# phylo42/IPK

Hardware: AMD Instinct MI355X
Metric: scored phylo-k-mers/sec (higher is better)
Workload: dtype f32

## Files before the change

ipk_amd/csrc/ipkgpu.hip:

```cpp
#include <cstring>
#include <hip/hip_runtime.h>
#include <rocprim/rocprim.hpp>

#include <algorithm>
#include <cmath>
#include <cstdarg>
#include <cstdio>
#include <cstring>
#include <new>
#include <string>
#include <type_traits>
#include <unordered_map>
#include <memory>
#include <vector>

#include "../../include/ipkgpu.h"
#include "dcla_device.hpp"
#include "kernels_score.hpp"
#include "kernels_quad.hpp"
#include "kernels_compact.hpp"
#include "kernels_keymajor.hpp"
#include "kernels_reduce_pipe.hpp"
#include "kernels_filter.hpp"
#include "kernels_dbfile.hpp"
#include <chrono>

using namespace ipkgpu;


namespace {

struct DevBuf {
    void* p = nullptr;
    size_t cap = 0;
    template <class T> T* as() const { return reinterpret_cast<T*>(p); }
};

struct EventPool {
    std::vector<hipEvent_t> free_ev;
    hipEvent_t get()
    {
        if (!free_ev.empty()) { hipEvent_t e = free_ev.back(); free_ev.pop_back(); return e; }
        hipEvent_t e = nullptr;
        return hipEventCreate(&e) == hipSuccess ? e : nullptr;
    }
    void put(hipEvent_t e) { if (free_ev.size() < 64) free_ev.push_back(e); else (void)hipEventDestroy(e); }
};
struct Stopwatch {
    hipStream_t stream;
    EventPool* pool;
    std::vector<hipEvent_t> ev;
    Stopwatch(hipStream_t s, EventPool* p) : stream(s), pool(p) {}
    ~Stopwatch() { for (hipEvent_t e : ev) pool->put(e); }
    int mark()
    {
        hipEvent_t e = pool->get();
        if (!e) return -1;
        (void)hipEventRecord(e, stream);
        ev.push_back(e);
        return (int)ev.size() - 1;
    }
    double ms(int a, int b) const
    {
        float t = 0;
        if (a < 0 || b < 0 || hipEventElapsedTime(&t, ev[a], ev[b]) != hipSuccess) return 0;
        return t;
    }
};

}

struct ipkgpu_comm;
struct ipkgpu_ctx;
static void ipkgpu_comm_release(ipkgpu_ctx* ctx);
struct ipkgpu_ctx {
    int device = 0;
    ipkgpu_comm* comm = nullptr;
    hipStream_t stream = nullptr;
    std::string err;
    int64_t workspace_bytes = 0;
    int64_t opt_variant = 0;
    int64_t opt_flags = 0;
    int64_t opt_kmc_pass = 0;
    int64_t opt_prefix_mats = 0;
    int64_t opt_wg_chunks2 = 0;
    int64_t opt_rounds = 0;
    int64_t opt_pool_limit = 0;
    int64_t opt_pool_chunks = 0;
    DevBuf table, best, ovfq, counts, offsets, goff, idx, branch, scan_sums, scan_boff, tmp_a, tmp_b, tmp_c;
    DevBuf pool, desc, gbcnt, gboff, gbcur, clist, gm, tile_next;
    DevBuf ptrs;
    DevBuf mask;
    bool mask_valid = false;
    uint64_t mask_words = 0;
    bool table_compressed = false;
    DevBuf rank, vaddr, ucnt, qpack, xstart, pcounts;
    DevBuf cvals, coff, croom;
    bool comp_own_vals = false;
    std::vector<uint32_t> h_branch;
    uint32_t comp_nb = 0, comp_stride = 0, comp_tbl = 0;
    double pairs_per_window = 0;
    double acc_main_ms = 0, acc_reduce_ms = 0;
    double acc_count_ms = 0, acc_write_ms = 0, acc_km_ms = 0;
    const char* main_kernel = "";
    std::vector<std::pair<void*, size_t>> free_blocks;
    std::unordered_map<void*, size_t> live_blocks;
    size_t cached_bytes = 0, cache_limit = 0;
    void* small = nullptr;
    void* h_up = nullptr; size_t h_up_cap = 0; hipEvent_t up_done = nullptr; bool up_pending = false;
    unsigned long long emitted_host = 0; bool emitted_fetched = false;
    uint32_t* h_rb = nullptr;
    EventPool events;
    bool spec_skip_wait = false;
    uint64_t pool_want_min = 0;
    struct Pending {
        bool active = false;
        std::unique_ptr<Stopwatch> sw; int ev_a = -1, ev_b = -1, ev_c = -1, ev_d = -1;
        uint64_t cap = 0, max_chunks = 0, windows = 0; uint32_t gb = 0; bool pool_ovf_ok = false, use_quad = false;
    } pend;
    uint64_t last_entries = 0; uint32_t last_gb = 0;
    double t_write_total = 0, t_write_device = 0, t_write_file = 0;
    int num_cu = 256;
};

struct ipkgpu_result {
    ipkgpu_ctx* ctx = nullptr;
    std::vector<uint32_t> group_ids;
    std::vector<uint64_t> offsets;
    uint64_t emitted = 0;
    uint32_t* d_keys = nullptr;
    float* d_scores = nullptr;
    uint32_t* d_positions = nullptr;
    size_t cap = 0;
    std::vector<uint32_t> h_keys;
    std::vector<float> h_scores;
    std::vector<uint32_t> h_positions;
    bool h_keys_ok = false, h_scores_ok = false, h_positions_ok = false;
    double t_total = 0, t_prefix = 0, t_score = 0, t_compact = 0, t_main = 0, t_reduce = 0;
    int score_launches = 0;
};

struct ipkgpu_parts {
    ipkgpu_ctx* ctx = nullptr;
    uint32_t n_owners = 1;
    uint64_t slots = 0;
    uint32_t* d_counts = nullptr;
    uint2* d_entries = nullptr;
    std::vector<uint64_t> owner_off;
    uint64_t emitted = 0;
    uint32_t* pre_keys = nullptr; uint64_t* pre_key_off = nullptr; uint64_t pre_n_keys = 0; double t_keys = 0;
    uint32_t lead = 0;
    uint64_t key_base = 0;
    double t_total = 0, t_prefix = 0, t_score = 0, t_compact = 0, t_main = 0, t_reduce = 0, t_count = 0, t_write = 0, t_km = 0;
    int score_launches = 0;
};

struct ipkgpu_db {
    ipkgpu_ctx* ctx = nullptr;
    uint64_t n_keys = 0, n_entries = 0;
    uint32_t* d_keys = nullptr;
    uint64_t* d_key_off = nullptr;
    uint2* d_entries = nullptr;
    std::vector<uint32_t> h_keys;
    std::vector<uint64_t> h_key_off;
    std::vector<uint32_t> h_entries;
    bool h_ok = false;
    double t_merge = 0;
    double* d_fv64 = nullptr;
    float* d_fv32 = nullptr;
    uint32_t* d_order = nullptr;
    std::vector<double> h_fv64;
    std::vector<float> h_fv32;
    std::vector<uint32_t> h_order;
    bool h_filter_ok = false;
    double t_filter = 0;
};

static std::string g_create_err;
constexpr size_t RB_BYTES = 4096, RB_OWNER_OFF = 8 , RB_OWNERS_MAX = 500;

template <class T = uint32_t> static T* small_at(const ipkgpu_ctx* ctx, uint32_t off) { return reinterpret_cast<T*>(static_cast<char*>(ctx->small) + off); }

static int fail(ipkgpu_ctx* ctx, int code, const char* fmt, ...)
{
    char buf[512];
    va_list ap;
    va_start(ap, fmt);
    vsnprintf(buf, sizeof buf, fmt, ap);
    va_end(ap);
    if (ctx) ctx->err = buf; else g_create_err = buf;
    return code;
}

#define HIP_TRY(ctx, expr)                                                                      \
    do {                                                                                        \
        hipError_t e_ = (expr);                                                                 \
        if (e_ != hipSuccess)                                                                   \
            return fail(ctx, e_ == hipErrorOutOfMemory ? IPKGPU_ERR_NOMEM : IPKGPU_ERR_HIP,     \
                        "%s failed: %s (%s:%d)", #expr, hipGetErrorString(e_), __FILE__, __LINE__); \
    } while (0)
#define RC_TRY(expr) do { int rc_ = (expr); if (rc_) return rc_; } while (0)

static int ensure(ipkgpu_ctx* ctx, DevBuf& b, size_t need)
{
    if (b.cap >= need && b.p) return IPKGPU_OK;
    const bool regrow = b.p != nullptr;
    if (b.p) { HIP_TRY(ctx, hipFree(b.p)); b.p = nullptr; b.cap = 0; }
    need = std::max<size_t>(need, 16);
    size_t want = regrow ? need + need / 16 : need;
    hipError_t e = hipMalloc(&b.p, want);
    if (e != hipSuccess && want > need) { (void)hipGetLastError(); want = need; e = hipMalloc(&b.p, want); }
    HIP_TRY(ctx, e);
    b.cap = want;
    return IPKGPU_OK;
}


static int upload_stage(ipkgpu_ctx* ctx, size_t bytes, void** out)
{
    if (ctx->up_pending) { HIP_TRY(ctx, hipEventSynchronize(ctx->up_done)); ctx->up_pending = false; }
    if (!ctx->up_done) HIP_TRY(ctx, hipEventCreateWithFlags(&ctx->up_done, hipEventDisableTiming));
    if (bytes > ctx->h_up_cap) {
        if (ctx->h_up) { (void)hipHostFree(ctx->h_up); ctx->h_up = nullptr; ctx->h_up_cap = 0; }
        const size_t cap = std::max<size_t>(bytes + bytes / 2, 1 << 16);
        HIP_TRY(ctx, hipHostMalloc(&ctx->h_up, cap, hipHostMallocDefault));
        ctx->h_up_cap = cap;
    }
    *out = ctx->h_up;
    return IPKGPU_OK;
}
static int upload_staged(ipkgpu_ctx* ctx)
{
    HIP_TRY(ctx, hipEventRecord(ctx->up_done, ctx->stream));
    ctx->up_pending = true;
    return IPKGPU_OK;
}

static hipError_t ctx_alloc(ipkgpu_ctx* ctx, void** out, size_t bytes)
{
    bytes = std::max<size_t>((bytes + 255) & ~(size_t)255, 256);
    size_t best = (size_t)-1;
    for (size_t i = 0; i < ctx->free_blocks.size(); ++i) {
        const size_t cap = ctx->free_blocks[i].second;
        if (cap >= bytes && cap <= bytes + bytes / 2 + (1 << 20) && (best == (size_t)-1 || cap < ctx->free_blocks[best].second)) best = i;
    }
    if (best != (size_t)-1) {
        *out = ctx->free_blocks[best].first;
        ctx->live_blocks[*out] = ctx->free_blocks[best].second;
        ctx->cached_bytes -= ctx->free_blocks[best].second;
        ctx->free_blocks.erase(ctx->free_blocks.begin() + best);
        return hipSuccess;
    }
    hipError_t e = hipMalloc(out, bytes);
    if (e != hipSuccess && !ctx->free_blocks.empty()) {
        for (auto& b : ctx->free_blocks) (void)hipFree(b.first);
        ctx->free_blocks.clear(); ctx->cached_bytes = 0;
        (void)hipGetLastError();
        e = hipMalloc(out, bytes);
    }
    if (e == hipSuccess) ctx->live_blocks[*out] = bytes;
    return e;
}
static void ctx_release(ipkgpu_ctx* ctx, void* p)
{
    if (!p) return;
    auto it = ctx->live_blocks.find(p);
    if (it == ctx->live_blocks.end()) { (void)hipFree(p); return; }
    const size_t cap = it->second;
    ctx->live_blocks.erase(it);
    if (ctx->cached_bytes + cap <= ctx->cache_limit) { ctx->free_blocks.push_back({p, cap}); ctx->cached_bytes += cap; }
    else (void)hipFree(p);
}

static constexpr uint64_t WAVE_PER_ITEM_SPAN = 1ull << 24;

static hipError_t ctx_alloc_atleast(ipkgpu_ctx* ctx, void** out, size_t min_bytes, size_t want_bytes, size_t* got)
{
    min_bytes = std::max<size_t>((min_bytes + 255) & ~(size_t)255, 256);
    want_bytes = std::max(want_bytes, min_bytes);
    size_t best = (size_t)-1;
    for (size_t i = 0; i < ctx->free_blocks.size(); ++i) {
        const size_t cap = ctx->free_blocks[i].second;
        if (cap >= min_bytes && cap <= want_bytes + want_bytes / 2 + (1 << 20) && (best == (size_t)-1 || cap < ctx->free_blocks[best].second)) best = i;
    }
    if (best != (size_t)-1) {
        *out = ctx->free_blocks[best].first;
        *got = ctx->free_blocks[best].second;
        ctx->live_blocks[*out] = *got;
        ctx->cached_bytes -= *got;
        ctx->free_blocks.erase(ctx->free_blocks.begin() + best);
        return hipSuccess;
    }
    const hipError_t e = ctx_alloc(ctx, out, want_bytes);
    if (e == hipSuccess) *got = ctx->live_blocks[*out];
    return e;
}

extern "C" {

uint32_t ipkgpu_bits_per_symbol(uint32_t sigma) { return sigma == 4 ? 2u : sigma == 20 ? 5u : 0u; }
uint32_t ipkgpu_max_k(uint32_t sigma) { return sigma == 4 ? 14u : sigma == 20 ? 6u : 0u; }
uint32_t ipkgpu_max_k_keyrange(uint32_t sigma) { return sigma == 4 ? 16u : ipkgpu_max_k(sigma); }
size_t ipkgpu_kmer_batch(uint32_t key, size_t n_ranges) { return n_ranges ? key % n_ranges : 0; }

float ipkgpu_log_threshold(float omega, uint32_t sigma, uint32_t k)
{
    return log10f(powf(omega / (float)sigma, (float)k));
}

const char* ipkgpu_last_error(const ipkgpu_ctx* ctx) { return ctx ? ctx->err.c_str() : g_create_err.c_str(); }

int ipkgpu_create(int device_id, ipkgpu_ctx** out)
{
    if (!out) return fail(nullptr, IPKGPU_ERR_INVALID, "ipkgpu_create: null out pointer");
    *out = nullptr;
    int n = 0;
    hipError_t e = hipGetDeviceCount(&n);
    if (e != hipSuccess || n <= 0)
        return fail(nullptr, IPKGPU_ERR_NODEVICE, "no HIP device available (%s); this engine has no CPU fallback",
                    e != hipSuccess ? hipGetErrorString(e) : "device count 0");
    if (device_id < 0 || device_id >= n)
        return fail(nullptr, IPKGPU_ERR_INVALID, "device %d out of range (0..%d)", device_id, n - 1);
    ipkgpu_ctx* ctx = new (std::nothrow) ipkgpu_ctx();
    if (!ctx) return fail(nullptr, IPKGPU_ERR_NOMEM, "out of host memory");
    ctx->device = device_id;
    if ((e = hipSetDevice(device_id)) != hipSuccess ||
        (e = hipStreamCreateWithFlags(&ctx->stream, hipStreamNonBlocking)) != hipSuccess) {
        delete ctx;
        return fail(nullptr, IPKGPU_ERR_HIP, "device setup failed: %s", hipGetErrorString(e));
    }
    hipDeviceProp_t prop;
    if (hipGetDeviceProperties(&prop, device_id) == hipSuccess) ctx->num_cu = prop.multiProcessorCount;
    size_t free_b = 0, total_b = 0;
    if (hipMemGetInfo(&free_b, &total_b) == hipSuccess) { ctx->workspace_bytes = (int64_t)(free_b / 2); ctx->cache_limit = free_b / 4; }
    else ctx->workspace_bytes = (int64_t)8 << 30;
    if ((e = hipMalloc(&ctx->small, SMALL_BYTES)) != hipSuccess) {
        (void)hipStreamDestroy(ctx->stream);
        delete ctx;
        return fail(nullptr, IPKGPU_ERR_NOMEM, "hipMalloc failed: %s", hipGetErrorString(e));
    }
    if ((e = hipHostMalloc((void**)&ctx->h_rb, RB_BYTES, hipHostMallocDefault)) != hipSuccess) {
        (void)hipFree(ctx->small);
        (void)hipStreamDestroy(ctx->stream);
        delete ctx;
        return fail(nullptr, IPKGPU_ERR_NOMEM, "hipHostMalloc failed: %s", hipGetErrorString(e));
    }
    memset(ctx->h_rb, 0, RB_BYTES);
    *out = ctx;
    return IPKGPU_OK;
}

void ipkgpu_destroy(ipkgpu_ctx* ctx)
{
    if (!ctx) return;
    (void)hipSetDevice(ctx->device);
    (void)hipStreamSynchronize(ctx->stream);
    DevBuf* bufs[] = {&ctx->table, &ctx->best, &ctx->ovfq, &ctx->counts, &ctx->offsets, &ctx->goff, &ctx->idx,
                      &ctx->branch, &ctx->scan_sums, &ctx->scan_boff, &ctx->tmp_a, &ctx->tmp_b, &ctx->tmp_c,
                      &ctx->pool, &ctx->desc, &ctx->gbcnt, &ctx->gboff, &ctx->gbcur, &ctx->clist, &ctx->gm, &ctx->tile_next, &ctx->mask,
                      &ctx->rank, &ctx->vaddr, &ctx->ucnt, &ctx->qpack, &ctx->xstart, &ctx->pcounts, &ctx->ptrs,
                      &ctx->cvals, &ctx->coff, &ctx->croom};
    for (DevBuf* b : bufs) if (b->p) (void)hipFree(b->p);
    for (auto& b : ctx->free_blocks) (void)hipFree(b.first);
    ipkgpu_comm_release(ctx);
    if (ctx->small) (void)hipFree(ctx->small);
    if (ctx->h_up) (void)hipHostFree(ctx->h_up);
    ctx->pend.sw.reset();
    for (hipEvent_t e : ctx->events.free_ev) (void)hipEventDestroy(e);
    ctx->events.free_ev.clear();
    if (ctx->h_rb) (void)hipHostFree(ctx->h_rb);
    if (ctx->up_done) (void)hipEventDestroy(ctx->up_done);
    (void)hipStreamDestroy(ctx->stream);
    delete ctx;
}

int ipkgpu_set_option(ipkgpu_ctx* ctx, const char* name, int64_t value)
{
    if (!ctx || !name) return IPKGPU_ERR_INVALID;
    if (!strcmp(name, "workspace_bytes")) {
        if (value <= 0) return fail(ctx, IPKGPU_ERR_INVALID, "workspace_bytes must be positive");
        ctx->workspace_bytes = value;
        return IPKGPU_OK;
    }
    if (!strcmp(name, "variant")) { ctx->opt_variant = value; return IPKGPU_OK; }
    if (!strcmp(name, "debug_flags")) { ctx->opt_flags = value; return IPKGPU_OK; }
    if (!strcmp(name, "debug_pool_chunks")) { ctx->opt_pool_chunks = value; return IPKGPU_OK; }
    if (!strcmp(name, "debug_pool_limit_bytes")) { ctx->opt_pool_limit = value; return IPKGPU_OK; }
    if (!strcmp(name, "debug_wg_chunks2")) { ctx->opt_wg_chunks2 = value; return IPKGPU_OK; }
    if (!strcmp(name, "debug_rounds")) { ctx->opt_rounds = value; return IPKGPU_OK; }
    if (!strcmp(name, "debug_kmc_pass")) { ctx->opt_kmc_pass = value; return IPKGPU_OK; }
    if (!strcmp(name, "debug_prefix_mats")) { ctx->opt_prefix_mats = value; return IPKGPU_OK; }
    return fail(ctx, IPKGPU_ERR_INVALID, "unknown option '%s'", name);
}

}

namespace {

constexpr int TW = 128;
constexpr int NW = 8;

#ifndef IPK_QCAP
#define IPK_QCAP 160
#endif
#ifndef IPK_AACAP
#define IPK_AACAP 512
#endif
#ifndef IPK_QCAP12
#define IPK_QCAP12 384
#endif
#ifndef IPK_QNW12
#define IPK_QNW12 4
#endif
#ifndef IPK_QTW12
#define IPK_QTW12 32
#endif
template <int SIGMA, int K> constexpr int fast_cap()
{
    if (SIGMA == 4) return K <= 10 ? IPK_QCAP : IPK_QCAP12;
    return IPK_AACAP;
}

template <int SIGMA, int K, bool POS = false>
int launch_score(ipkgpu_ctx* ctx, const ScoreParams& p)
{
    constexpr int CAP = fast_cap<SIGMA, K>();
    constexpr size_t lds = TileGeo<SIGMA, K, TW>::HEAD_BYTES + (size_t)NW * wave_scratch_entries<SIGMA, K, CAP>() * 8;
    static_assert(lds <= 160 * 1024, "fast-path LDS budget");
    auto kern = score_tiles_kernel<SIGMA, K, CAP, TW, NW, POS>;
    if (lds > 64 * 1024)
        HIP_TRY(ctx, hipFuncSetAttribute(reinterpret_cast<const void*>(kern), hipFuncAttributeMaxDynamicSharedMemorySize, (int)lds));
    const uint64_t blocks = (uint64_t)p.n_batch_mats * p.tiles_per_mat;
    if (blocks > 0x7fffffffull) return fail(ctx, IPKGPU_ERR_INVALID, "batch too large for one launch");
    hipLaunchKernelGGL(kern, dim3((uint32_t)blocks), dim3(NW * 64), lds, ctx->stream, p);
    HIP_TRY(ctx, hipGetLastError());
    return IPKGPU_OK;
}

template <int SIGMA, int K, bool POS = false>
int launch_overflow(ipkgpu_ctx* ctx, const ScoreParams& p)
{
    if constexpr (Geo<SIGMA, K, 1 << 30>::DIRECT || ipow(SIGMA, K - K / 2) <= (uint32_t)fast_cap<SIGMA, K>()) {
        (void)ctx; (void)p;
        return IPKGPU_OK;
    } else {
        constexpr size_t lds = TileGeo<SIGMA, K, 1>::HEAD_BYTES + (size_t)wave_scratch_entries<SIGMA, K, big_capf<SIGMA, K>()>() * 8;
        static_assert(lds <= 160 * 1024, "big-list LDS budget");
        auto kern = score_overflow_kernel<SIGMA, K, POS>;
        if (lds > 64 * 1024)
            HIP_TRY(ctx, hipFuncSetAttribute(reinterpret_cast<const void*>(kern), hipFuncAttributeMaxDynamicSharedMemorySize, (int)lds));
        const uint32_t per_cu = (uint32_t)std::max<size_t>(1, std::min<size_t>(32 / OVF_NW, (160 * 1024) / (lds + 64)));
        hipLaunchKernelGGL(kern, dim3(ctx->num_cu * per_cu), dim3(OVF_NW * 64), lds, ctx->stream, p);
        HIP_TRY(ctx, hipGetLastError());
        return IPKGPU_OK;
    }
}

template <int SIGMA, int K, bool POS>
int launch_both(ipkgpu_ctx* ctx, const ScoreParams& p)
{
    RC_TRY((launch_score<SIGMA, K, POS>(ctx, p)));
    return launch_overflow<SIGMA, K, POS>(ctx, p);
}


template <int SIGMA, int K> constexpr uint32_t stream_tbl()
{
    constexpr uint64_t T = ipow(SIGMA, K);
    if (Geo<SIGMA, K, 1 << 30>::DIRECT) return 0;
    if (SIGMA == 4 && K >= 13) return 0;
    if (SIGMA == 4) return T <= 16384 ? (uint32_t)T : (K <= 10 ? 16384u : 32768u);
    if (K <= 3) return (uint32_t)T;
    if (K <= 5) return 32000u;
    return 0;
}

template <int SIGMA, int K> constexpr int stream_nw() { return NW; }
template <int SIGMA, int K> constexpr int stream_tw() { return TW; }

template <int SIGMA, int K>
int launch_stream_pass1(ipkgpu_ctx* ctx, const StreamParams& sp, uint32_t n_wg)
{
    constexpr uint32_t TBL = stream_tbl<SIGMA, K>();
    if constexpr (TBL == 0) { (void)sp; (void)n_wg; return fail(ctx, IPKGPU_ERR_INVALID, "stream variant unsupported for this sigma/k"); }
    else {
        constexpr int CAP = fast_cap<SIGMA, K>();
        constexpr uint32_t T = ipow(SIGMA, K);
        constexpr uint32_t NB = (T + TBL - 1) / TBL;
        constexpr int SNW = stream_nw<SIGMA, K>(), STW = stream_tw<SIGMA, K>();
        constexpr size_t lds = TileGeo<SIGMA, K, STW>::HEAD_BYTES + (size_t)SNW * stream_wave_scratch<SIGMA, K, CAP>() * 8 + (size_t)SNW * 2 * NB * SUB * 4;
        static_assert(lds <= 160 * 1024, "stream pass-1 LDS budget");
        auto kern = score_stream_kernel<SIGMA, K, CAP, STW, SNW, TBL>;
        if (lds > 64 * 1024)
            HIP_TRY(ctx, hipFuncSetAttribute(reinterpret_cast<const void*>(kern), hipFuncAttributeMaxDynamicSharedMemorySize, (int)lds));
        hipLaunchKernelGGL(kern, dim3(n_wg), dim3(SNW * 64), lds, ctx->stream, sp);
        HIP_TRY(ctx, hipGetLastError());
        return IPKGPU_OK;
    }
}

template <int SIGMA, int K>
int launch_stream_overflow(ipkgpu_ctx* ctx, const StreamParams& sp)
{
    constexpr uint32_t TBL = stream_tbl<SIGMA, K>();
    if constexpr (TBL == 0 || ipow(SIGMA, K - K / 2) <= (uint32_t)fast_cap<SIGMA, K>()) {
        (void)ctx; (void)sp;
        return IPKGPU_OK;
    } else {
        constexpr uint32_t NB = (uint32_t)((ipow(SIGMA, K) + TBL - 1) / TBL);
        constexpr size_t lds = TileGeo<SIGMA, K, 1>::HEAD_BYTES + (size_t)wave_scratch_entries<SIGMA, K, big_capf<SIGMA, K>()>() * 8 +
                               (size_t)OVF_NW * 2 * NB * SUB * 4;
        static_assert(lds + 64 <= 160 * 1024, "big-list (stream) LDS budget");
        auto kern = score_overflow_stream_kernel<SIGMA, K, TBL>;
        if (lds > 64 * 1024)
            HIP_TRY(ctx, hipFuncSetAttribute(reinterpret_cast<const void*>(kern), hipFuncAttributeMaxDynamicSharedMemorySize, (int)lds));
        const uint32_t per_cu = (uint32_t)std::max<size_t>(1, std::min<size_t>(32 / OVF_NW, (160 * 1024) / (lds + 64)));
        hipLaunchKernelGGL(kern, dim3(ctx->num_cu * per_cu), dim3(OVF_NW * 64), lds, ctx->stream, sp);
        HIP_TRY(ctx, hipGetLastError());
        return IPKGPU_OK;
    }
}

#ifndef IPK_RPIPE_DEFAULT
#define IPK_RPIPE_DEFAULT 1
#endif
#ifndef IPK_RPIPE_D
#define IPK_RPIPE_D 2
#endif
template <int SIGMA, int K>
int launch_stream_pass2(ipkgpu_ctx* ctx, uint32_t n_gb, uint64_t T, uint32_t* table, bool compress)
{
    constexpr uint32_t TBL = stream_tbl<SIGMA, K>();
    if constexpr (TBL == 0) { (void)n_gb; (void)T; (void)table; (void)compress; return fail(ctx, IPKGPU_ERR_INVALID, "stream variant unsupported"); }
    else {
        constexpr uint32_t NB = (uint32_t)((ipow(SIGMA, K) + TBL - 1) / TBL);
        constexpr int NT = TBL <= 16384 ? 512 : 1024;
        const size_t lds = compress ? (size_t)comp_padded_slots<TBL, NT>() * 4 + (NT / 64 + 1) * 4 : (size_t)TBL * 4;
        auto launch = [&](auto kern) -> int {
            if (lds > 64 * 1024)
                HIP_TRY(ctx, hipFuncSetAttribute(reinterpret_cast<const void*>(kern), hipFuncAttributeMaxDynamicSharedMemorySize, (int)lds));
            hipLaunchKernelGGL(kern, dim3(n_gb), dim3(NT), lds, ctx->stream, ctx->pool.as<uint2>(),
                               ctx->gboff.as<uint64_t>(), ctx->clist.as<uint2>(), NB, T, table, ctx->mask.as<uint32_t>(), ctx->mask_words,
                               ctx->cvals.as<uint2>(), ctx->coff.as<uint64_t>(), ctx->rank.as<uint32_t>(), ctx->vaddr.as<uint64_t>(), ctx->ucnt.as<uint32_t>());
            HIP_TRY(ctx, hipGetLastError());
            return IPKGPU_OK;
        };
        if constexpr (TBL * 4 > 80 * 1024) {
            if (compress && ((IPK_RPIPE_DEFAULT != 0) != ((ctx->opt_flags & 2048) != 0))) {
                constexpr int PD = IPK_RPIPE_D;
                auto kern = reduce_buckets_pipe_kernel<TBL, NT, PD>;
                HIP_TRY(ctx, hipFuncSetAttribute(reinterpret_cast<const void*>(kern), hipFuncAttributeMaxDynamicSharedMemorySize, (int)lds));
                hipLaunchKernelGGL(kern, dim3(std::min<uint32_t>(n_gb, (uint32_t)ctx->num_cu)), dim3(NT), lds, ctx->stream, ctx->pool.as<uint2>(),
                                   ctx->gboff.as<uint64_t>(), ctx->clist.as<uint2>(), n_gb, NB, T, ctx->mask.as<uint32_t>(), ctx->mask_words,
                                   ctx->cvals.as<uint2>(), ctx->coff.as<uint64_t>(), ctx->rank.as<uint32_t>(), ctx->vaddr.as<uint64_t>(), ctx->ucnt.as<uint32_t>());
                HIP_TRY(ctx, hipGetLastError());
                return IPKGPU_OK;
            }
        }
        return compress ? launch(reduce_buckets_kernel<TBL, NT, true>) : launch(reduce_buckets_kernel<TBL, NT, false>);
    }
}

template <int SIGMA, int K> size_t stream_lds() {
    constexpr uint32_t TBL = stream_tbl<SIGMA, K>();
    if constexpr (TBL == 0) return 0;
    else {
        constexpr int CAP = fast_cap<SIGMA, K>();
        constexpr uint32_t NB = (uint32_t)((ipow(SIGMA, K) + TBL - 1) / TBL);
        return TileGeo<SIGMA, K, stream_tw<SIGMA, K>()>::HEAD_BYTES + (size_t)stream_nw<SIGMA, K>() * stream_wave_scratch<SIGMA, K, CAP>() * 8 +
               (size_t)stream_nw<SIGMA, K>() * 2 * NB * SUB * 4;
    }
}
template <int SIGMA, int K> uint32_t stream_nb() {
    constexpr uint32_t TBL = stream_tbl<SIGMA, K>();
    if constexpr (TBL == 0) return 0; else return (uint32_t)((ipow(SIGMA, K) + TBL - 1) / TBL);
}

template <int SIGMA, int K> constexpr bool quad_ok() { return QuadGeo<SIGMA, K>::OK && stream_tbl<SIGMA, K>() != 0; }
#ifndef IPK_QNW
#define IPK_QNW 4
#endif
#ifndef IPK_QTW
#define IPK_QTW 40
#endif
template <int SIGMA, int K> constexpr int quad_nw() { return K <= 10 ? IPK_QNW : IPK_QNW12; }
template <int SIGMA, int K> constexpr int quad_tw() { return K <= 10 ? IPK_QTW : IPK_QTW12; }
#ifndef IPK_QROWLANE12
#define IPK_QROWLANE12 1
#endif
#ifndef IPK_QROWLANE
#define IPK_QROWLANE 0
#endif
template <int SIGMA, int K> constexpr bool quad_rowlane() { return K <= 10 ? IPK_QROWLANE != 0 : IPK_QROWLANE12 != 0; }
#ifndef IPK_QONEWIN12
#define IPK_QONEWIN12 1
#endif
template <int SIGMA, int K> constexpr bool quad_onewin() { return K >= 11 && IPK_QONEWIN12 != 0 && quad_rowlane<SIGMA, K>(); }
template <int SIGMA, int K> size_t quad_lds()
{
    if constexpr (!quad_ok<SIGMA, K>()) return 0;
    else {
        constexpr int CAP = fast_cap<SIGMA, K>();
        constexpr uint32_t TBL = stream_tbl<SIGMA, K>();
        constexpr uint32_t NB = (uint32_t)((ipow(SIGMA, K) + TBL - 1) / TBL);
        return QuadTile<SIGMA, K, quad_tw<SIGMA, K>()>::HEAD_BYTES + (size_t)quad_nw<SIGMA, K>() * quad_wave_entries<SIGMA, K, CAP, quad_onewin<SIGMA, K>()>() * 8 +
               (size_t)quad_nw<SIGMA, K>() * NB * 8;
    }
}
template <int SIGMA, int K, bool COUNT_ONLY = false>
int launch_quad_pass1(ipkgpu_ctx* ctx, const StreamParams& sp, uint32_t n_wg)
{
    if constexpr (!quad_ok<SIGMA, K>()) { (void)sp; (void)n_wg; return fail(ctx, IPKGPU_ERR_INVALID, "quad kernel unsupported for this sigma/k"); }
    else {
        constexpr int CAP = fast_cap<SIGMA, K>();
        constexpr uint32_t TBL = stream_tbl<SIGMA, K>();
        constexpr int QNW = quad_nw<SIGMA, K>(), QTW = quad_tw<SIGMA, K>();
        const size_t lds = quad_lds<SIGMA, K>();
        auto kern = score_quad_kernel<SIGMA, K, CAP, QTW, QNW, TBL, COUNT_ONLY, quad_rowlane<SIGMA, K>(), quad_onewin<SIGMA, K>()>;
        if (lds > 64 * 1024)
            HIP_TRY(ctx, hipFuncSetAttribute(reinterpret_cast<const void*>(kern), hipFuncAttributeMaxDynamicSharedMemorySize, (int)lds));
        hipLaunchKernelGGL(kern, dim3(n_wg), dim3(QNW * 64), lds, ctx->stream, sp);
        HIP_TRY(ctx, hipGetLastError());
        return IPKGPU_OK;
    }
}

#ifndef IPK_XPNW
#define IPK_XPNW 11
#endif
#ifndef IPK_XPTW
#define IPK_XPTW 128
#endif
constexpr int XP_TW = IPK_XPTW;
template <int SIGMA, int K> constexpr int xp_nw() { return SIGMA == 20 ? IPK_XPNW : 11; }
template <int SIGMA, int K> constexpr uint32_t xp_tbl()
{
    if (SIGMA == 20 && K == 6) return 16000u;
    if (SIGMA == 4 && K >= 13) return 32768u;
    return stream_tbl<SIGMA, K>();
}
template <int SIGMA, int K, int KK = K> uint32_t xp_nb() {
    constexpr uint32_t TBL = xp_tbl<SIGMA, K>();
    if constexpr (TBL == 0) return 0; else return (uint32_t)((ipow(SIGMA, KK) + TBL - 1) / TBL);
}
template <int SIGMA, int K, int KK = K> size_t xp_lds() {
    constexpr uint32_t TBL = xp_tbl<SIGMA, K>();
    if constexpr (TBL == 0) return 0;
    else {
        constexpr int CAP = fast_cap<SIGMA, K>();
        constexpr uint32_t NB = (uint32_t)((ipow(SIGMA, KK) + TBL - 1) / TBL);
        return TileGeo<SIGMA, K, XP_TW>::HEAD_BYTES + (size_t)xp_nw<SIGMA, K>() * stream_wave_scratch<SIGMA, K, CAP>() * 8 + (size_t)NB * 4;
    }
}
template <int SIGMA, int K, bool WRITE, int KK = K>
int launch_xp(ipkgpu_ctx* ctx, const XpParams& xp, uint32_t n_wg)
{
    constexpr uint32_t TBL = xp_tbl<SIGMA, K>();
    if constexpr (TBL == 0) { (void)xp; (void)n_wg; return fail(ctx, IPKGPU_ERR_INVALID, "exact-partition variant unsupported for this sigma/k"); }
    else {
        constexpr int CAP = fast_cap<SIGMA, K>();
        constexpr uint32_t NB = (uint32_t)((ipow(SIGMA, KK) + TBL - 1) / TBL);
        constexpr size_t lds = TileGeo<SIGMA, K, XP_TW>::HEAD_BYTES + (size_t)xp_nw<SIGMA, K>() * stream_wave_scratch<SIGMA, K, CAP>() * 8 + (size_t)NB * 4;
        static_assert(lds <= 160 * 1024, "exact-partition LDS budget");
        static_assert((TileGeo<SIGMA, K, XP_TW>::HEAD_BYTES + (size_t)xp_nw<SIGMA, K>() * stream_wave_scratch<SIGMA, K, CAP>() * 8) % 8 == 0, "cursor alignment");
        auto kern = score_xp_kernel<SIGMA, K, CAP, XP_TW, xp_nw<SIGMA, K>(), TBL, WRITE, KK>;
        if (lds > 64 * 1024)
            HIP_TRY(ctx, hipFuncSetAttribute(reinterpret_cast<const void*>(kern), hipFuncAttributeMaxDynamicSharedMemorySize, (int)lds));
        hipLaunchKernelGGL(kern, dim3(n_wg), dim3(xp_nw<SIGMA, K>() * 64), lds, ctx->stream, xp);
        HIP_TRY(ctx, hipGetLastError());
        return IPKGPU_OK;
    }
}
template <int SIGMA, int K, bool WRITE, int KK = K>
int launch_xp_overflow(ipkgpu_ctx* ctx, const XpParams& xp)
{
    constexpr uint32_t TBL = xp_tbl<SIGMA, K>();
    if constexpr (TBL == 0 || ipow(SIGMA, K - K / 2) <= (uint32_t)fast_cap<SIGMA, K>()) {
        (void)ctx; (void)xp;
        return IPKGPU_OK;
    } else {
        constexpr size_t lds = TileGeo<SIGMA, K, 1>::HEAD_BYTES + (size_t)wave_scratch_entries<SIGMA, K, big_capf<SIGMA, K>()>() * 8;
        static_assert(lds + 64 <= 160 * 1024, "big-list (exact partition) LDS budget");
        auto kern = score_overflow_xp_kernel<SIGMA, K, TBL, WRITE, KK>;
        if (lds > 64 * 1024)
            HIP_TRY(ctx, hipFuncSetAttribute(reinterpret_cast<const void*>(kern), hipFuncAttributeMaxDynamicSharedMemorySize, (int)lds));
        const uint32_t per_cu = (uint32_t)std::max<size_t>(1, std::min<size_t>(32 / OVF_NW, (160 * 1024) / (lds + 64)));
        hipLaunchKernelGGL(kern, dim3(ctx->num_cu * per_cu), dim3(OVF_NW * 64), lds, ctx->stream, xp);
        HIP_TRY(ctx, hipGetLastError());
        return IPKGPU_OK;
    }
}
template <int SIGMA, int K, bool COMPRESS, int KK = K>
int launch_xp_reduce(ipkgpu_ctx* ctx, uint32_t n_gb, uint32_t S, uint64_t T, const uint64_t* off, uint32_t* table)
{
    constexpr uint32_t TBL = xp_tbl<SIGMA, K>();
    if constexpr (TBL == 0) { (void)n_gb; (void)S; (void)T; (void)off; (void)table; return fail(ctx, IPKGPU_ERR_INVALID, "exact-partition variant unsupported"); }
    else {
        constexpr uint32_t NB = (uint32_t)((ipow(SIGMA, KK) + TBL - 1) / TBL);
        static_assert(!COMPRESS || NB == 1 || TBL % 64 == 0, "a 64-slot block must not straddle two buckets");
        constexpr int NT = TBL <= 16384 ? 512 : 1024;
        constexpr size_t lds = COMPRESS ? (size_t)comp_padded_slots<TBL, NT>() * 4 + (NT / 64 + 1) * 4 : (size_t)TBL * 4;
        auto kern = reduce_ranges_kernel<TBL, NT, COMPRESS>;
        if (lds > 64 * 1024)
            HIP_TRY(ctx, hipFuncSetAttribute(reinterpret_cast<const void*>(kern), hipFuncAttributeMaxDynamicSharedMemorySize, (int)lds));
        hipLaunchKernelGGL(kern, dim3(n_gb), dim3(NT), lds, ctx->stream, ctx->pool.as<uint2>(), off, S, NB, T, table,
                           ctx->mask.as<uint32_t>(), ctx->mask_words, ctx->rank.as<uint32_t>(), ctx->vaddr.as<uint64_t>(), ctx->ucnt.as<uint32_t>());
        HIP_TRY(ctx, hipGetLastError());
        return IPKGPU_OK;
    }
}
template <int V> using int_c = std::integral_constant<int, V>;

template <int SIGMA, int K, int KMAX, class F> int with_k(ipkgpu_ctx* ctx, uint32_t k, F& f)
{
    if (k == (uint32_t)K) return f(int_c<SIGMA>{}, int_c<K>{});
    if constexpr (K < KMAX) return with_k<SIGMA, K + 1, KMAX>(ctx, k, f);
    else return fail(ctx, IPKGPU_ERR_INVALID, "unsupported sigma/k (%u/%u)", (uint32_t)SIGMA, k);
}
template <class F> int with_sigma_k(ipkgpu_ctx* ctx, uint32_t sigma, uint32_t k, F&& f)
{
    if (sigma == 4) return with_k<4, 2, 14>(ctx, k, f);
    if (sigma == 20) return with_k<20, 2, 6>(ctx, k, f);
    return fail(ctx, IPKGPU_ERR_INVALID, "unsupported sigma/k (%u/%u)", sigma, k);
}

bool keyrange_supported(uint32_t sigma, uint32_t k, uint32_t lead)
{
    return sigma == 4 && lead >= 1 && k > lead && k - lead >= 13 && k - lead <= 14 && k <= 16;
}
template <class F> int with_xp_shape(ipkgpu_ctx* ctx, uint32_t sigma, uint32_t k, uint32_t lead, F&& f)
{
    if (!lead) return with_sigma_k(ctx, sigma, k, [&](auto S_, auto K_) { return f(S_, K_, K_); });
    if (sigma == 4) {
        switch (k * 8 + lead) {
            case 14 * 8 + 1: return f(int_c<4>{}, int_c<14>{}, int_c<13>{});
            case 15 * 8 + 1: return f(int_c<4>{}, int_c<15>{}, int_c<14>{});
            case 15 * 8 + 2: return f(int_c<4>{}, int_c<15>{}, int_c<13>{});
            case 16 * 8 + 2: return f(int_c<4>{}, int_c<16>{}, int_c<14>{});
            case 16 * 8 + 3: return f(int_c<4>{}, int_c<16>{}, int_c<13>{});
        }
    }
    return fail(ctx, IPKGPU_ERR_INVALID, "unsupported key range");
}

struct Geometry {
    uint32_t fast_cap = 0;
    uint32_t stream_nb = 0, stream_tbl = 0;
    uint32_t stream_nw = NW, stream_tw = TW;
    size_t stream_lds = 0;
    bool quad = false;
    uint32_t quad_nw = NW, quad_tw = TW;
    size_t quad_lds = 0;
    uint32_t xp_nb = 0, xp_tbl = 0;
    size_t xp_lds = 0;
};

int fill_geometry(ipkgpu_ctx* ctx, uint32_t sigma, uint32_t k, uint32_t lead, Geometry& g)
{
    if (!lead)
        RC_TRY(with_sigma_k(ctx, sigma, k, [&](auto S_, auto K_) {
            g.fast_cap = fast_cap<S_, K_>();
            g.stream_nb = stream_nb<S_, K_>(); g.stream_tbl = stream_tbl<S_, K_>();
            g.stream_nw = stream_nw<S_, K_>(); g.stream_tw = stream_tw<S_, K_>(); g.stream_lds = stream_lds<S_, K_>();
            g.quad = quad_ok<S_, K_>();
            g.quad_nw = quad_nw<S_, K_>(); g.quad_tw = quad_tw<S_, K_>(); g.quad_lds = quad_lds<S_, K_>();
            return IPKGPU_OK;
        }));
    return with_xp_shape(ctx, sigma, k, lead, [&](auto S_, auto K_, auto KK_) {
        g.xp_nb = xp_nb<S_, K_, KK_>(); g.xp_tbl = xp_tbl<S_, K_>(); g.xp_lds = xp_lds<S_, K_, KK_>();
        return IPKGPU_OK;
    });
}

#ifndef IPK_KMC_RUNS_DEFAULT
#define IPK_KMC_RUNS_DEFAULT 1
#endif
#ifndef IPK_KMC_PASS
#define IPK_KMC_PASS 256
#endif
#define KM_LAUNCH(KERN, CAPV, ...)                                                                                        \
    do {                                                                                                                  \
        if (P == 1) hipLaunchKernelGGL((KERN<true, CAPV>), dim3((uint32_t)(per_xcd * 8)), dim3(256), 0, ctx->stream, __VA_ARGS__); \
        else hipLaunchKernelGGL((KERN<false, CAPV>), dim3((uint32_t)(per_xcd * 8)), dim3(256), 0, ctx->stream, __VA_ARGS__);     \
    } while (0)

CompTable comp_table(const ipkgpu_ctx* ctx)
{
    CompTable ct;
    ct.mask = ctx->mask.as<uint32_t>(); ct.rank = ctx->rank.as<uint32_t>(); ct.vaddr = ctx->vaddr.as<uint64_t>();
    ct.pool = ctx->comp_own_vals ? ctx->cvals.as<uint2>() : ctx->pool.as<uint2>();
    ct.off = ctx->comp_own_vals ? ctx->coff.as<uint64_t>() : ctx->gboff.as<uint64_t>(); ct.mask_words = ctx->mask_words;
    ct.NB = ctx->comp_nb; ct.stride = ctx->comp_stride; ct.TBL = ctx->comp_tbl;
    return ct;
}

}

namespace {

constexpr int IPKGPU_RETRY_SMALLER = 100;
constexpr int IPKGPU_RETRY_AGAIN = 101;
#ifndef IPK_OVF_POOL_RATIO
#define IPK_OVF_POOL_RATIO 500
#endif

enum class PassKind { tiles, stream, quad, xp };
struct Pass {
    PassKind kind = PassKind::tiles;
    bool positions = false;
    bool compress = false;
    double slot_bytes() const { return positions ? 8.0 : kind == PassKind::xp && compress ? 0.3125 : 4.0; }
};

Pass choose_pass(int64_t variant, uint32_t sigma, uint32_t lead, bool positions, const Geometry& g)
{
    Pass ps;
    ps.positions = positions;
    if (positions) return ps;
    const int64_t v = variant;
    if (g.xp_nb != 0 && (v == 3 || v == 4 || (v == 0 && g.stream_nb == 0) || lead != 0)) {
        ps.kind = PassKind::xp;
        ps.compress = v != 3;
    } else if (g.stream_nb != 0 && g.stream_nb <= 2048 && (v == 0 || v == 2 || v == 5 || v == 6 || v == 7)) {
        ps.kind = v != 2 && g.quad ? PassKind::quad : PassKind::stream;
        ps.compress = v == 6 || (v == 0 && g.stream_tbl == 32768u && sigma == 4);
    }
    return ps;
}

struct Plan {
    uint32_t n_mats = 0, sites = 0, sigma = 0, k = 0;
    float eps = 0;
    std::vector<uint32_t> group_ids;
    std::vector<uint32_t> slot_of;
    uint32_t n_groups = 0, nwin = 0, tiles_per_mat = 0, chunks_per_group = 0;
    uint64_t table_size = 0, gpb = 1;
    uint32_t lead = 0, lead_c = 0;
    Geometry geo;
    Pass pass;
    const uint32_t* mat_rank = nullptr;
};

int make_plan(ipkgpu_ctx* ctx, const void* logp, uint32_t n_mats, uint32_t sites, uint32_t sigma,
              const uint32_t* mat_group, uint32_t k, float log_eps, Plan& pl, uint32_t lead = 0, uint32_t lead_c = 0,
              bool positions = false)
{
    if (!logp || !mat_group) return fail(ctx, IPKGPU_ERR_INVALID, "null input pointer");
    if (sigma != 4 && sigma != 20) return fail(ctx, IPKGPU_ERR_INVALID, "unsupported alphabet size %u (4 or 20)", sigma);
    if (lead == 0 && (k < 2 || k > ipkgpu_max_k(sigma)))
        return fail(ctx, IPKGPU_ERR_INVALID, "k=%u out of range [2, %u] for sigma=%u", k, ipkgpu_max_k(sigma), sigma);
    if (lead != 0 && !keyrange_supported(sigma, k, lead))
        return fail(ctx, IPKGPU_ERR_INVALID, "no key-range pass of k=%u with %u leading symbols for sigma=%u", k, lead, sigma);
    pl.lead = lead; pl.lead_c = lead_c;
    if (n_mats == 0) return fail(ctx, IPKGPU_ERR_INVALID, "no matrices");
    if (sites < k) return fail(ctx, IPKGPU_ERR_INVALID, "alignment has %u sites, fewer than k=%u", sites, k);
    pl.n_mats = n_mats; pl.sites = sites; pl.sigma = sigma; pl.k = k; pl.eps = log_eps;
    RC_TRY(fill_geometry(ctx, sigma, k, lead, pl.geo));
    pl.pass = choose_pass(ctx->opt_variant, sigma, lead, positions, pl.geo);
    pl.slot_of.resize(n_mats);
// ... 1636 lines not shown
```

ipk_amd/csrc/kernels_reduce_pipe.hpp:

```cpp
#pragma once
#include "kernels_score.hpp"
#include "kernels_keymajor.hpp"

namespace ipkgpu {

template <uint32_t TBL, int NT, int D>
__global__ __launch_bounds__(NT) void reduce_buckets_pipe_kernel(const uint2* __restrict__ pool, const uint64_t* __restrict__ off,
                                                                 const uint2* __restrict__ list, uint32_t n_gb, uint32_t NB, uint64_t T,
                                                                 uint32_t* __restrict__ mask, uint64_t mask_words,
                                                                 uint2* __restrict__ cvals, const uint64_t* __restrict__ coff,
                                                                 uint32_t* __restrict__ rank, uint64_t* __restrict__ vaddr,
                                                                 uint32_t* __restrict__ ucnt)
{
    constexpr uint32_t CH = chunk_pairs<TBL>();
    constexpr int PER = CH / 64;
    constexpr uint32_t NWV = NT / 64, PAD = comp_padded_slots<TBL, NT>();
    extern __shared__ __align__(16) unsigned char smem[];
    uint32_t* tab = reinterpret_cast<uint32_t*>(smem);
    const uint32_t lane = lane_id(), wave = (uint32_t)__builtin_amdgcn_readfirstlane((int)(threadIdx.x >> 6));
    const uint32_t G = gridDim.x, first = blockIdx.x;
    if (first >= n_gb) return;
    const uint32_t n_items = (n_gb - first + G - 1) / G;

    struct Meta { uint32_t c0, n; };
    auto load_meta = [&](uint32_t x) {
        Meta m{0u, 0u};
        if (x < n_items) {
            const uint32_t gb = first + x * G;
            const uint64_t o0 = uniform_load(off + gb), o1 = uniform_load(off + gb + 1);
            m.c0 = (uint32_t)o0; m.n = (uint32_t)(o1 - o0);
        }
        return m;
    };
    auto load_cv = [&](uint32_t x) { return x < n_items ? uniform_load(coff + (first + x * G)) : 0ull; };
    auto share = [&](const Meta& m, uint32_t& start, uint32_t& cnt) {
        const uint32_t q = m.n / NWV, r = m.n % NWV;
        cnt = q + (wave < r ? 1u : 0u);
        start = m.c0 + wave * q + min(wave, r);
    };
    struct Desc { uint2 e[D]; };
    static_assert(D == 2 || D == 4 || D == 8, "a trip's descriptors are one s_load_dwordx{4,8,16}");
    auto load_desc = [&](uint32_t idx) {
        Desc d;
        const uint64_t* p = reinterpret_cast<const uint64_t*>(list + idx);
#pragma unroll
        for (int j = 0; j < D; ++j) { const uint64_t w = uniform_load(p + j); d.e[j] = make_uint2((uint32_t)w, (uint32_t)(w >> 32)); }
        return d;
    };

    uint32_t cur = 0, lpos = 0, cstart, ccnt;
    Meta mcur = load_meta(0), mnext = load_meta(1), min2 = load_meta(2);
    share(mcur, cstart, ccnt);
    uint32_t ntake = min((uint32_t)D, ccnt), nkind = ccnt <= (uint32_t)D ? 2u : 1u;
    Desc nd = load_desc(cstart);
    uint64_t cv = load_cv(0), cvn = load_cv(1);

    uint32_t it = 0;
    uint32_t k0 = 0;

    auto fill = [&](uint2 (&P)[D * PER], uint32_t (&pc)[D]) -> uint32_t {
        const uint32_t kind = nkind, take = ntake;
#pragma unroll
        for (int j = 0; j < D; ++j) {
            const bool ok = (uint32_t)j < take;
            const uint32_t id = ok ? nd.e[j].x : 0u, cnt = ok ? nd.e[j].y : 0u;
            pc[j] = cnt;
            const uint2* s = pool + (size_t)id * CH;
#pragma unroll
            for (int q = 0; q < PER; ++q) {
                const uint2* sq = s + ((uint32_t)(64 * q) < cnt ? 64u * q : 0u);
                P[j * PER + q] = pool_load(sq + lane);
            }
        }
        lpos += take;
        if (kind == 2) {
            ++cur; lpos = 0;
            mcur = mnext; mnext = min2; min2 = load_meta(cur + 2);
            share(mcur, cstart, ccnt);
        }
        if (kind != 0 && cur < n_items) {
            ntake = min((uint32_t)D, ccnt - lpos);
            nkind = lpos + ntake >= ccnt ? 2u : 1u;
            nd = load_desc(cstart + lpos);
        } else {
            ntake = 0; nkind = 0;
        }
        return kind;
    };
    auto consume = [&](const uint2 (&P)[D * PER], const uint32_t (&pc)[D]) {
#pragma unroll
        for (int j = 0; j < D; ++j)
#pragma unroll
            for (int q = 0; q < PER; ++q)
                if (lane + 64u * q < pc[j]) atomicMax(&tab[P[j * PER + q].x - k0], enc_score_bits(P[j * PER + q].y));
    };
    auto boundary = [&]() {
        __syncthreads();
        const uint32_t gb = first + it * G;
        const uint32_t g = gb / NB, b = gb - g * NB;
        const uint64_t key0 = (uint64_t)b * TBL;
        const uint32_t nslots = (uint32_t)min((uint64_t)TBL, T - key0);
        compress_slice<TBL, NT, true, true>(tab, nslots, reinterpret_cast<uint32_t*>(cvals + cv), mask + (size_t)g * mask_words + (key0 >> 5),
                                            rank + (size_t)g * (mask_words / 2) + (key0 >> 6), vaddr + (size_t)g * (mask_words / 2) + (key0 >> 6), ucnt + gb);
        __syncthreads();
        ++it;
        cv = cvn; cvn = load_cv(it + 1);
        const uint32_t gbn = first + it * G;
        k0 = (gbn % NB) * TBL;
    };

    k0 = (first % NB) * TBL;
    uint2 PA[D * PER], PB[D * PER];
    uint32_t pcA[D], pcB[D];
    uint32_t kA = fill(PA, pcA), kB = fill(PB, pcB);
    for (uint32_t i = threadIdx.x; i < PAD / 4; i += NT) reinterpret_cast<uint4*>(tab)[i] = make_uint4(0, 0, 0, 0);
    __syncthreads();
    consume(PA, pcA);
    bool endA = kA == 2;
    for (;;) {
        kA = fill(PA, pcA);
        if (endA) { boundary(); if (it >= n_items) break; }
        consume(PB, pcB);
        const bool endB = kB == 2;
        kB = fill(PB, pcB);
        if (endB) { boundary(); if (it >= n_items) break; }
        consume(PA, pcA);
        endA = kA == 2;
    }
}

}
```

Baseline: 132.0 billion.

## Extend pipelined persistent reduce kernel to dense output and 16K-slot tables

The pipelined persistent bucket-reduce kernel, which double-buffers pool loads across slices, was previously used only for compressed output with large LDS tables. It now also handles the dense (uncompressed) epilogue through a new dense_slice_out that copies the LDS slice to the table, stores the mask and clears LDS. It is also enabled for TBL 16384, launched at two blocks per CU. The aim is to hide global-load latency and cut the per-bucket launch and reinit cost of the non-pipelined reduce kernel. Debug knobs for grid size, descriptor depth and absent-lane load variants are added, and smaller slices risk lower occupancy or load imbalance in exchange.

```diff
diff --git a/ipk_amd/csrc/ipkgpu.hip b/ipk_amd/csrc/ipkgpu.hip
--- a/ipk_amd/csrc/ipkgpu.hip
+++ b/ipk_amd/csrc/ipkgpu.hip
@@ -85,6 +85,7 @@
     int64_t opt_prefix_mats = 0;
     int64_t opt_wg_chunks2 = 0;
     int64_t opt_rounds = 0;
+    int64_t opt_reduce_grid = 0;
     int64_t opt_pool_limit = 0;
     int64_t opt_pool_chunks = 0;
     DevBuf table, best, ovfq, counts, offsets, goff, idx, branch, scan_sums, scan_boff, tmp_a, tmp_b, tmp_c;
@@ -388,6 +389,7 @@
     if (!strcmp(name, "debug_pool_limit_bytes")) { ctx->opt_pool_limit = value; return IPKGPU_OK; }
     if (!strcmp(name, "debug_wg_chunks2")) { ctx->opt_wg_chunks2 = value; return IPKGPU_OK; }
     if (!strcmp(name, "debug_rounds")) { ctx->opt_rounds = value; return IPKGPU_OK; }
+    if (!strcmp(name, "debug_reduce_grid")) { ctx->opt_reduce_grid = value; return IPKGPU_OK; }
     if (!strcmp(name, "debug_kmc_pass")) { ctx->opt_kmc_pass = value; return IPKGPU_OK; }
     if (!strcmp(name, "debug_prefix_mats")) { ctx->opt_prefix_mats = value; return IPKGPU_OK; }
     return fail(ctx, IPKGPU_ERR_INVALID, "unknown option '%s'", name);
@@ -527,6 +529,12 @@
 #ifndef IPK_RPIPE_D
 #define IPK_RPIPE_D 2
 #endif
+#ifndef IPK_RPIPE_D64
+#define IPK_RPIPE_D64 2
+#endif
+#ifndef IPK_RPIPE_MIN_SLICES
+#define IPK_RPIPE_MIN_SLICES 0
+#endif
 template <int SIGMA, int K>
 int launch_stream_pass2(ipkgpu_ctx* ctx, uint32_t n_gb, uint64_t T, uint32_t* table, bool compress)
 {
@@ -545,16 +553,26 @@
             HIP_TRY(ctx, hipGetLastError());
             return IPKGPU_OK;
         };
-        if constexpr (TBL * 4 > 80 * 1024) {
-            if (compress && ((IPK_RPIPE_DEFAULT != 0) != ((ctx->opt_flags & 2048) != 0))) {
-                constexpr int PD = IPK_RPIPE_D;
-                auto kern = reduce_buckets_pipe_kernel<TBL, NT, PD>;
-                HIP_TRY(ctx, hipFuncSetAttribute(reinterpret_cast<const void*>(kern), hipFuncAttributeMaxDynamicSharedMemorySize, (int)lds));
-                hipLaunchKernelGGL(kern, dim3(std::min<uint32_t>(n_gb, (uint32_t)ctx->num_cu)), dim3(NT), lds, ctx->stream, ctx->pool.as<uint2>(),
-                                   ctx->gboff.as<uint64_t>(), ctx->clist.as<uint2>(), n_gb, NB, T, ctx->mask.as<uint32_t>(), ctx->mask_words,
-                                   ctx->cvals.as<uint2>(), ctx->coff.as<uint64_t>(), ctx->rank.as<uint32_t>(), ctx->vaddr.as<uint64_t>(), ctx->ucnt.as<uint32_t>());
-                HIP_TRY(ctx, hipGetLastError());
-                return IPKGPU_OK;
+        constexpr bool PIPE_COMP = TBL * 4 > 80 * 1024 || TBL == 16384, PIPE_DENSE = TBL == 16384 || TBL == 32768;
+        if constexpr (PIPE_COMP || PIPE_DENSE) {
+            const bool by_rule = (TBL * 4 > 80 * 1024 && compress) || n_gb >= (uint32_t)IPK_RPIPE_MIN_SLICES;
+            if ((compress ? PIPE_COMP : PIPE_DENSE) && ((IPK_RPIPE_DEFAULT != 0 && by_rule) != ((ctx->opt_flags & 2048) != 0))) {
+                constexpr int PD = TBL == 16384 ? IPK_RPIPE_D64 : IPK_RPIPE_D;
+                const uint32_t per_cu = TBL * 4 > 80 * 1024 ? 1u : 2u;
+                uint32_t grid = std::min<uint32_t>(n_gb, (uint32_t)ctx->num_cu * per_cu);
+                if (ctx->opt_reduce_grid > 0) grid = std::min<uint32_t>(n_gb, (uint32_t)ctx->opt_reduce_grid);
+                auto pipe = [&](auto kern) -> int {
+                    if (lds > 64 * 1024)
+                        HIP_TRY(ctx, hipFuncSetAttribute(reinterpret_cast<const void*>(kern), hipFuncAttributeMaxDynamicSharedMemorySize, (int)lds));
+                    hipLaunchKernelGGL(kern, dim3(grid), dim3(NT), lds, ctx->stream, ctx->pool.as<uint2>(),
+                                       ctx->gboff.as<uint64_t>(), ctx->clist.as<uint2>(), n_gb, NB, T, ctx->mask.as<uint32_t>(), ctx->mask_words,
+                                       ctx->cvals.as<uint2>(), ctx->coff.as<uint64_t>(), ctx->rank.as<uint32_t>(), ctx->vaddr.as<uint64_t>(), ctx->ucnt.as<uint32_t>(),
+                                       table);
+                    HIP_TRY(ctx, hipGetLastError());
+                    return IPKGPU_OK;
+                };
+                if constexpr (PIPE_COMP) if (compress) return pipe(reduce_buckets_pipe_kernel<TBL, NT, PD, true>);
+                if constexpr (PIPE_DENSE) if (!compress) return pipe(reduce_buckets_pipe_kernel<TBL, NT, PD, false>);
             }
         }
         return compress ? launch(reduce_buckets_kernel<TBL, NT, true>) : launch(reduce_buckets_kernel<TBL, NT, false>);
diff --git a/ipk_amd/csrc/kernels_reduce_pipe.hpp b/ipk_amd/csrc/kernels_reduce_pipe.hpp
--- a/ipk_amd/csrc/kernels_reduce_pipe.hpp
+++ b/ipk_amd/csrc/kernels_reduce_pipe.hpp
@@ -2,19 +2,40 @@
 #include "kernels_score.hpp"
 #include "kernels_keymajor.hpp"
 
+#ifndef IPK_RPIPE_ABSENT64
+#define IPK_RPIPE_ABSENT64 0
+#endif
+
 namespace ipkgpu {
 
-template <uint32_t TBL, int NT, int D>
+template <uint32_t TBL, int NT>
+__device__ __forceinline__ void dense_slice_out(uint32_t* tab, uint32_t* dst, uint32_t* mrow)
+{
+    constexpr uint32_t NWV = NT / 64, SPW = TBL / NWV;
+    static_assert(TBL % (NWV * 256) == 0, "whole 64-lane 16-byte rows per wavefront");
+    const uint32_t lane = lane_id(), wave = (uint32_t)__builtin_amdgcn_readfirstlane((int)(threadIdx.x >> 6));
+    uint4* src = reinterpret_cast<uint4*>(tab + wave * SPW) + lane;
+    uint4* out = reinterpret_cast<uint4*>(dst + wave * SPW) + lane;
+#pragma unroll
+    for (uint32_t q = 0; q < SPW / 256; ++q) out[64 * q] = src[64 * q];
+    store_slice_mask(tab, TBL, mrow, NT);
+#pragma unroll
+    for (uint32_t q = 0; q < SPW / 256; ++q) src[64 * q] = make_uint4(0, 0, 0, 0);
+}
+
+template <uint32_t TBL, int NT, int D, bool COMPRESS = true>
 __global__ __launch_bounds__(NT) void reduce_buckets_pipe_kernel(const uint2* __restrict__ pool, const uint64_t* __restrict__ off,
                                                                  const uint2* __restrict__ list, uint32_t n_gb, uint32_t NB, uint64_t T,
                                                                  uint32_t* __restrict__ mask, uint64_t mask_words,
                                                                  uint2* __restrict__ cvals, const uint64_t* __restrict__ coff,
                                                                  uint32_t* __restrict__ rank, uint64_t* __restrict__ vaddr,
-                                                                 uint32_t* __restrict__ ucnt)
+                                                                 uint32_t* __restrict__ ucnt, uint32_t* __restrict__ table)
 {
+    static_assert(COMPRESS || TBL == 16384 || TBL == 32768, "dense epilogue: whole, aligned slices only");
     constexpr uint32_t CH = chunk_pairs<TBL>();
     constexpr int PER = CH / 64;
-    constexpr uint32_t NWV = NT / 64, PAD = comp_padded_slots<TBL, NT>();
+    constexpr int ABSENT = TBL == 16384 ? IPK_RPIPE_ABSENT64 : 0;
+    constexpr uint32_t NWV = NT / 64, PAD = COMPRESS ? comp_padded_slots<TBL, NT>() : TBL;
     extern __shared__ __align__(16) unsigned char smem[];
     uint32_t* tab = reinterpret_cast<uint32_t*>(smem);
     const uint32_t lane = lane_id(), wave = (uint32_t)__builtin_amdgcn_readfirstlane((int)(threadIdx.x >> 6));
@@ -32,14 +53,17 @@
         }
         return m;
     };
-    auto load_cv = [&](uint32_t x) { return x < n_items ? uniform_load(coff + (first + x * G)) : 0ull; };
+    auto load_cv = [&](uint32_t x) {
+        if constexpr (COMPRESS) return x < n_items ? uniform_load(coff + (first + x * G)) : 0ull;
+        else return 0ull;
+    };
     auto share = [&](const Meta& m, uint32_t& start, uint32_t& cnt) {
         const uint32_t q = m.n / NWV, r = m.n % NWV;
         cnt = q + (wave < r ? 1u : 0u);
         start = m.c0 + wave * q + min(wave, r);
     };
     struct Desc { uint2 e[D]; };
-    static_assert(D == 2 || D == 4 || D == 8, "a trip's descriptors are one s_load_dwordx{4,8,16}");
+    static_assert(D == 1 || D == 2 || D == 4 || D == 8, "a trip's descriptors are one s_load_dwordx{2,4,8,16}");
     auto load_desc = [&](uint32_t idx) {
         Desc d;
         const uint64_t* p = reinterpret_cast<const uint64_t*>(list + idx);
@@ -68,8 +92,14 @@
             const uint2* s = pool + (size_t)id * CH;
 #pragma unroll
             for (int q = 0; q < PER; ++q) {
-                const uint2* sq = s + ((uint32_t)(64 * q) < cnt ? 64u * q : 0u);
-                P[j * PER + q] = pool_load(sq + lane);
+                if constexpr (ABSENT == 2) {
+                    if (lane + 64u * q < cnt) P[j * PER + q] = pool_load(s + 64u * q + lane);
+                } else if constexpr (ABSENT == 3) {
+                    P[j * PER + q] = pool_load(s + (lane + 64u * q < cnt ? lane + 64u * q : 0u));
+                } else {
+                    const uint2* sq = ABSENT == 1 ? ((uint32_t)(64 * q) < cnt ? s + 64u * q : pool) : s + ((uint32_t)(64 * q) < cnt ? 64u * q : 0u);
+                    P[j * PER + q] = pool_load(sq + lane);
+                }
             }
         }
         lpos += take;
@@ -99,9 +129,12 @@
         const uint32_t gb = first + it * G;
         const uint32_t g = gb / NB, b = gb - g * NB;
         const uint64_t key0 = (uint64_t)b * TBL;
-        const uint32_t nslots = (uint32_t)min((uint64_t)TBL, T - key0);
-        compress_slice<TBL, NT, true, true>(tab, nslots, reinterpret_cast<uint32_t*>(cvals + cv), mask + (size_t)g * mask_words + (key0 >> 5),
-                                            rank + (size_t)g * (mask_words / 2) + (key0 >> 6), vaddr + (size_t)g * (mask_words / 2) + (key0 >> 6), ucnt + gb);
+        if constexpr (COMPRESS) {
+            const uint32_t nslots = (uint32_t)min((uint64_t)TBL, T - key0);
+            compress_slice<TBL, NT, true, true>(tab, nslots, reinterpret_cast<uint32_t*>(cvals + cv), mask + (size_t)g * mask_words + (key0 >> 5),
+                                                rank + (size_t)g * (mask_words / 2) + (key0 >> 6), vaddr + (size_t)g * (mask_words / 2) + (key0 >> 6), ucnt + gb);
+        } else
+            dense_slice_out<TBL, NT>(tab, table + (size_t)g * T + key0, mask + (size_t)g * mask_words + (key0 >> 5));
         __syncthreads();
         ++it;
         cv = cvn; cvn = load_cv(it + 1);
```

New measurement: 129.0 billion. 2.2% lower.
